# broadinstitute/Tangram

Measured on NVIDIA B200. Metric: map_cells_to_space iterations/sec, higher is better.
Workload: dtype bf16 operands / f32 accumulate+state

## Files before the change

tangram_b200/csrc/gemm_tc.cuh:

```cuda
#pragma once
#include <cuda.h>
#include <cstdio>
#include "common.cuh"
#include "gemm_simt.cuh"

namespace tgb {

constexpr int TC_BM = 128;
constexpr int TC_BK = 64;
constexpr int TC_UMMA_K = 16;
constexpr int TC_THREADS = 192;
constexpr int TC_RDOT_BN = 256;

__device__ __forceinline__ uint32_t smem_u32(const void* p) { return (uint32_t)__cvta_generic_to_shared(p); }

__device__ __forceinline__ void mbar_init(uint64_t* bar, uint32_t count) {
  asm volatile("mbarrier.init.shared::cta.b64 [%0], %1;" ::"r"(smem_u32(bar)), "r"(count));
}
__device__ __forceinline__ void mbar_expect_tx(uint64_t* bar, uint32_t bytes) {
  asm volatile("mbarrier.arrive.expect_tx.shared::cta.b64 _, [%0], %1;" ::"r"(smem_u32(bar)), "r"(bytes) : "memory");
}
__device__ __forceinline__ void mbar_wait(uint64_t* bar, uint32_t parity) {
  asm volatile(
      "{\n\t.reg .pred p;\n\t"
// ... 339 lines not shown
    }
  } else if (warp == 1) {
    if (lane == 0) {
      uint32_t kbg = 0;
      int it = 0;
      for (int w = blockIdx.x; w < total; w += gridDim.x, ++it) {
        const int z = w / (tiles_n * tiles_m);
        const int k_begin = k_off + z * k_per_split;
        const int k_end = min(k_total, k_begin + k_per_split);
        const int num_kb = (k_end - k_begin + TC_BK - 1) / TC_BK;
        const int b = it & 1;
        mbar_wait(&tempty_bar[b], (((uint32_t)it >> 1) & 1) ^ 1);
        tc_fence_after();
        const uint32_t d_tmem = tmem_base + (uint32_t)(b * BN);
        const int total_kb = num_kb * n_pairs;
        for (int kb = 0; kb < total_kb; ++kb, ++kbg) {
          const int s = kbg % STAGES;
          const uint32_t ph = (kbg / STAGES) & 1;
          mbar_wait(&full_bar[s], ph);
          tc_fence_after();
          const uint32_t sa = smem_u32(smem + s * kStageBytes);
          const uint32_t sb = sa + TileA::kBytes;
#pragma unroll
          for (int k = 0; k < TC_BK / TC_UMMA_K; ++k)
            umma_bf16(d_tmem, TileA::desc(sa, k), TileB::desc(sb, k), kIdesc, (kb > 0 || k > 0) ? 1u : 0u);
          umma_commit(&empty_bar[s]);
        }
        umma_commit(&tfull_bar[b]);
      }
    }
  } else {
    const int q = warp & 3;
    const int ew = warp - 2;
    int it = 0;
    for (int w = blockIdx.x; w < total; w += gridDim.x, ++it) {
      TileCoord t;
      t.split = w / (tiles_n * tiles_m);
      int tm_i;
      tile_mn(w - t.split * tiles_n * tiles_m, tiles_m, tiles_n, group_m, tm_i, t.tile_n);
      t.tiles_n = tiles_n;
      t.n0 = t.tile_n * BN;
      t.m0 = (tm_off + tm_i) * TC_BM;
      const int b = it & 1;
#ifndef TGB_SKIP_EPI
      epi.template prologue<BN, EPI_WARPS>(t, q, ew, lane);
#endif
      mbar_wait(&tfull_bar[b], ((uint32_t)it >> 1) & 1);
      tc_fence_after();
#ifndef TGB_SKIP_EPI
      epi.template run<BN, EPI_WARPS>(tmem_base + (uint32_t)(b * BN), q, ew, lane, t);
#endif
      tc_fence_before();
      __syncwarp();
      if (lane == 0) mbar_arrive(&tempty_bar[b]);
    }
    epi.finish(ew, lane, 0);
  }
  tc_fence_before();
  __syncthreads();
  if (warp == 1) tmem_dealloc(tmem_base, kTmemCols);
}

__device__ __forceinline__ uint32_t cluster_ctarank() {
  uint32_t r;
  asm volatile("mov.u32 %0, %%cluster_ctarank;" : "=r"(r));
  return r;
}
__device__ __forceinline__ void cluster_sync_all() {
  asm volatile("barrier.cluster.arrive.release.aligned;\n\tbarrier.cluster.wait.acquire.aligned;" ::: "memory");
}
__device__ __forceinline__ uint32_t mapa_shared(uint32_t addr, uint32_t rank) {
  uint32_t r;
  asm volatile("mapa.shared::cluster.u32 %0, %1, %2;" : "=r"(r) : "r"(addr), "r"(rank));
  return r;
}
__device__ __forceinline__ void mbar_arrive_remote(uint32_t cluster_addr) {
  asm volatile("mbarrier.arrive.release.cluster.shared::cluster.b64 _, [%0];" ::"r"(cluster_addr) : "memory");
}
__device__ __forceinline__ void tma_load_2d_pair(const CUtensorMap* map, uint32_t leader_bar, uint32_t dst, int c0, int c1, uint64_t policy) {
  asm volatile(
      "cp.async.bulk.tensor.2d.cta_group::2.shared::cluster.global.mbarrier::complete_tx::bytes.L2::cache_hint [%0], [%1, {%3, %4}], [%2], %5;"
      ::"r"(dst), "l"(map), "r"(leader_bar), "r"(c0), "r"(c1), "l"(policy) : "memory");
}
__device__ __forceinline__ void umma_bf16_pair(uint32_t d_tmem, uint64_t a_desc, uint64_t b_desc, uint32_t idesc, uint32_t accumulate) {
  asm volatile(
      "{\n\t.reg .pred p;\n\t"
      "setp.ne.b32 p, %4, 0;\n\t"
      "tcgen05.mma.cta_group::2.kind::f16 [%0], %1, %2, %3, p;\n\t}"
      ::"r"(d_tmem), "l"(a_desc), "l"(b_desc), "r"(idesc), "r"(accumulate) : "memory");
}
__device__ __forceinline__ void umma_commit_pair(uint64_t* bar) {
  asm volatile("tcgen05.commit.cta_group::2.mbarrier::arrive::one.shared::cluster.multicast::cluster.b64 [%0], %1;"
               ::"r"(smem_u32(bar)), "h"((uint16_t)3) : "memory");
}
__device__ __forceinline__ void tmem_alloc_pair(uint32_t* dst_smem, uint32_t ncols) {
  asm volatile("tcgen05.alloc.cta_group::2.sync.aligned.shared::cta.b32 [%0], %1;" ::"r"(smem_u32(dst_smem)), "r"(ncols) : "memory");
  asm volatile("tcgen05.relinquish_alloc_permit.cta_group::2.sync.aligned;" ::: "memory");
}
__device__ __forceinline__ void tmem_dealloc_pair(uint32_t taddr, uint32_t ncols) {
  asm volatile("tcgen05.dealloc.cta_group::2.sync.aligned.b32 %0, %1;" ::"r"(taddr), "r"(ncols) : "memory");
}

template <int BN, int STAGES, int EPI_WARPS, class Epi>
__global__ void __launch_bounds__(64 + 32 * EPI_WARPS, 1)
k_gemm_tc_pair(const __grid_constant__ TcMaps maps_a, const __grid_constant__ TcMaps maps_b, int n_pairs, int k_total, int tiles_m, int tiles_n, int group_m,
               uint64_t policy_a, uint64_t policy_b, int tm_off, const Epi epi) {
  using TileA = OperandTile<true, TC_BM>;
  using TileB = OperandTile<true, BN / 2>;
  constexpr int kStageBytes = TileA::kBytes + TileB::kBytes;
  constexpr uint32_t kTmemCols = 2 * BN;
  static_assert(kTmemCols == 256 || kTmemCols == 512, "TMEM allocation must be a power of two <= 512");
  constexpr uint32_t kIdesc = make_idesc(2 * TC_BM, BN, false, false);

  extern __shared__ uint8_t smem_raw[];
  uint8_t* smem = reinterpret_cast<uint8_t*>(((uintptr_t)smem_raw + 1023) & ~(uintptr_t)1023);
  __shared__ __align__(8) uint64_t full_bar[STAGES];
  __shared__ __align__(8) uint64_t empty_bar[STAGES];
  __shared__ __align__(8) uint64_t tfull_bar[2];
  __shared__ __align__(8) uint64_t tempty_bar[2];
  __shared__ uint32_t tmem_base_smem;

  const int warp = threadIdx.x >> 5, lane = threadIdx.x & 31;
  const uint32_t rank = cluster_ctarank();
  const int cid = blockIdx.x >> 1, ncl = gridDim.x >> 1;
  const int total = tiles_m * tiles_n;
  const int num_kb = (k_total + TC_BK - 1) / TC_BK;

  if (warp == 0 && lane == 0) {
    tma_prefetch_desc(&maps_a.m[0]);
    tma_prefetch_desc(&maps_b.m[0]);
#pragma unroll
    for (int s = 0; s < STAGES; ++s) { mbar_init(&full_bar[s], 1); mbar_init(&empty_bar[s], 1); }
#pragma unroll
    for (int b = 0; b < 2; ++b) { mbar_init(&tfull_bar[b], 1); mbar_init(&tempty_bar[b], 2 * EPI_WARPS); }
    fence_barrier_init();
  }
  if (warp == 1) tmem_alloc_pair(&tmem_base_smem, kTmemCols);
  tc_fence_before();
  cluster_sync_all();
  tc_fence_after();
  const uint32_t tmem_base = tmem_base_smem;

  if (warp == 0) {
#ifdef TGB_SKIP_MAINLOOP
    if (false) {
#else
    if (lane == 0) {
#endif
      uint32_t kbg = 0;
      for (int w = cid; w < total; w += ncl) {
        int tm_i, tn_i;
        tile_mn(w, tiles_m, tiles_n, group_m, tm_i, tn_i);
        const int n0 = tn_i * BN + (int)rank * (BN / 2);
        const int m0 = (tm_off + tm_i) * (2 * TC_BM) + (int)rank * TC_BM;
        for (int pr = 6 - n_pairs; pr < 6; ++pr) {
          const CUtensorMap* ma = &maps_a.m[kPairA[pr]];
          const CUtensorMap* mb = &maps_b.m[kPairB[pr]];
          for (int kb = 0; kb < num_kb; ++kb, ++kbg) {
            const int s = kbg % STAGES;
            const uint32_t ph = (kbg / STAGES) & 1;
            mbar_wait(&empty_bar[s], ph ^ 1);
            const uint32_t sa = smem_u32(smem + s * kStageBytes);
            const uint32_t sb = sa + TileA::kBytes;
            if (rank == 0) mbar_expect_tx(&full_bar[s], 2 * kStageBytes);
            const uint32_t lbar = mapa_shared(smem_u32(&full_bar[s]), 0);
            tma_load_2d_pair(ma, lbar, sa, kb * TC_BK, m0, policy_a);
            tma_load_2d_pair(mb, lbar, sb, kb * TC_BK, n0, policy_b);
          }
        }
      }
    }
  } else if (warp == 1) {
    if (lane == 0 && rank == 0) {
      uint32_t kbg = 0;
      int it = 0;
      for (int w = cid; w < total; w += ncl, ++it) {
        const int b = it & 1;
        mbar_wait(&tempty_bar[b], (((uint32_t)it >> 1) & 1) ^ 1);
        tc_fence_after();
        const uint32_t d_tmem = tmem_base + (uint32_t)(b * BN);
#ifdef TGB_SKIP_MAINLOOP
        const int total_kb = 0;
#else
        const int total_kb = num_kb * n_pairs;
#endif
        for (int kb = 0; kb < total_kb; ++kb, ++kbg) {
          const int s = kbg % STAGES;
          const uint32_t ph = (kbg / STAGES) & 1;
          mbar_wait(&full_bar[s], ph);
          tc_fence_after();
          const uint32_t sa = smem_u32(smem + s * kStageBytes);
          const uint32_t sb = sa + TileA::kBytes;
#pragma unroll
          for (int k = 0; k < TC_BK / TC_UMMA_K; ++k)
            umma_bf16_pair(d_tmem, TileA::desc(sa, k), TileB::desc(sb, k), kIdesc, (kb > 0 || k > 0) ? 1u : 0u);
          umma_commit_pair(&empty_bar[s]);
        }
        umma_commit_pair(&tfull_bar[b]);
      }
    }
  } else {
    const int q = warp & 3;
    const int ew = warp - 2;
    const uint32_t tempty_remote = mapa_shared(smem_u32(&tempty_bar[0]), 0);
    int it = 0;
    for (int w = cid; w < total; w += ncl, ++it) {
      TileCoord t;
      int tm_i;
      tile_mn(w, tiles_m, tiles_n, group_m, tm_i, t.tile_n);
      t.tiles_n = tiles_n;
      t.n0 = t.tile_n * BN;
      t.m0 = (tm_off + tm_i) * (2 * TC_BM) + (int)rank * TC_BM;
      t.split = 0;
      const int b = it & 1;
#ifndef TGB_SKIP_EPI
      epi.template prologue<BN, EPI_WARPS>(t, q, ew, lane);
#endif
      mbar_wait(&tfull_bar[b], ((uint32_t)it >> 1) & 1);
      tc_fence_after();
#ifndef TGB_SKIP_EPI
      epi.template run<BN, EPI_WARPS>(tmem_base + (uint32_t)(b * BN), q, ew, lane, t);
#endif
      tc_fence_before();
      __syncwarp();
      if (lane == 0) mbar_arrive_remote(tempty_remote + (uint32_t)b * 8u);
    }
    epi.finish(ew, lane, 0);
  }
  tc_fence_before();
  cluster_sync_all();
  if (warp == 1) tmem_dealloc_pair(tmem_base, kTmemCols);
}

typedef CUresult (*PFN_encodeTiled)(CUtensorMap*, CUtensorMapDataType, cuuint32_t, void*, const cuuint64_t*,
                                    const cuuint64_t*, const cuuint32_t*, const cuuint32_t*, CUtensorMapInterleave,
                                    CUtensorMapSwizzle, CUtensorMapL2promotion, CUtensorMapFloatOOBfill);

struct TcContext {
  PFN_encodeTiled encode = nullptr;
  int num_sms = 148;
  int pair_clusters = -1;
  int dp_clusters = -1;
  const void* smem_fn[16] = {};
  int smem_bytes[16] = {};
};

static inline int tc_init(TcContext& tc, char* err, size_t n) {
  void* fn = nullptr;
  cudaDriverEntryPointQueryResult qres;
  cudaError_t e = cudaGetDriverEntryPoint("cuTensorMapEncodeTiled", &fn, cudaEnableDefault, &qres);
  if (e != cudaSuccess || fn == nullptr || qres != cudaDriverEntryPointSuccess) {
    snprintf(err, n, "cuTensorMapEncodeTiled not available from the driver (%s)", cudaGetErrorString(e));
    return -2;
  }
  tc.encode = (PFN_encodeTiled)fn;
  int dev = 0;
  cudaGetDevice(&dev);
  cudaDeviceGetAttribute(&tc.num_sms, cudaDevAttrMultiProcessorCount, dev);
  return 0;
}

static inline int tc_make_map(TcContext& tc, CUtensorMap* map, const void* base, uint64_t cols, uint64_t rows,
                              uint64_t ld, uint32_t box_inner, uint32_t box_outer, char* err, size_t n) {
  cuuint64_t dims[2] = {cols, rows};
  cuuint64_t strides[1] = {ld * 2};
  cuuint32_t box[2] = {box_inner, box_outer};
  cuuint32_t estr[2] = {1, 1};
  CUresult r = tc.encode(map, CU_TENSOR_MAP_DATA_TYPE_BFLOAT16, 2, const_cast<void*>(base), dims, strides, box, estr,
                         CU_TENSOR_MAP_INTERLEAVE_NONE, CU_TENSOR_MAP_SWIZZLE_128B, CU_TENSOR_MAP_L2_PROMOTION_L2_256B,
                         CU_TENSOR_MAP_FLOAT_OOB_FILL_NONE);
  if (r != CUDA_SUCCESS) {
    snprintf(err, n, "cuTensorMapEncodeTiled failed (%d) cols=%llu rows=%llu ld=%llu box=%ux%u", (int)r,
             (unsigned long long)cols, (unsigned long long)rows, (unsigned long long)ld, box_inner, box_outer);
    return -2;
  }
  return 0;
}

template <class Kern>
static inline int tc_set_smem(TcContext& tc, Kern kern, int bytes, char* err, size_t n) {
  const void* key = reinterpret_cast<const void*>(kern);
  int slot = -1;
  for (int i = 0; i < 16; ++i) {
    if (tc.smem_fn[i] == key) { if (tc.smem_bytes[i] == bytes) return 0; slot = i; break; }
    if (tc.smem_fn[i] == nullptr && slot < 0) slot = i;
  }
  cudaError_t e = cudaFuncSetAttribute(kern, cudaFuncAttributeMaxDynamicSharedMemorySize, bytes);
  if (e != cudaSuccess) { snprintf(err, n, "cudaFuncSetAttribute(smem=%d): %s", bytes, cudaGetErrorString(e)); return -2; }
  if (slot >= 0) { tc.smem_fn[slot] = key; tc.smem_bytes[slot] = bytes; }
  return 0;
}
static inline int tc_check_launch(const char* name, char* err, size_t n) {
  cudaError_t e = cudaGetLastError();
  if (e != cudaSuccess) { snprintf(err, n, "launch %s: %s", name, cudaGetErrorString(e)); return -2; }
  return 0;
}

constexpr int TC_FWD_BN = 256, TC_FWD_STAGES = 4;
#ifndef TGB_BWD_BN
#define TGB_BWD_BN 256
#endif
constexpr int TC_BWD_BN = TGB_BWD_BN;
#ifndef TGB_BWD_PAIR
#define TGB_BWD_PAIR 1
#endif
constexpr int TC_PAIR_MIN_ROWS = 2048;
#ifndef TGB_DP_STAGES
#define TGB_DP_STAGES 6
#endif
#ifndef TGB_DP_EPI_WARPS
#define TGB_DP_EPI_WARPS 4
#endif
constexpr int TC_DP_STAGES = TGB_DP_STAGES, TC_DP_SINGLE_STAGES = 4, TC_DP_EPI_WARPS = TGB_DP_EPI_WARPS;
static inline int tc_dp_row_parts(int V) { return (int)ceil_div(V, TC_BWD_BN) * (TC_DP_EPI_WARPS / 4); }
static inline int tc_splits(long long tiles, long long k_total, int min_k) {
  long long s = (2 * 148 + tiles - 1) / tiles;
  const long long max_s = (k_total + min_k - 1) / min_k;
  if (s > max_s) s = max_s;
  if (s < 1) s = 1;
  const long long kps = ((k_total + s - 1) / s + TC_BK - 1) / TC_BK * TC_BK;
  return (int)((k_total + kps - 1) / kps);
}
static inline int tc_splits_for_chain(long long k_total, int max_chain) {
  long long s = (k_total + max_chain - 1) / max_chain;
  if (s < 1) s = 1;
  const long long kps = ((k_total + s - 1) / s + TC_BK - 1) / TC_BK * TC_BK;
  return (int)((k_total + kps - 1) / kps);
}
static inline int tc_forward_splits(int N, int V, int Ke) {
  return tc_splits((long long)ceil_div(V, TC_BM) * ceil_div(Ke, TC_FWD_BN), N, 512);
}
static inline int tc_kps(int k_total, int splits) {
  return (int)(round_up(ceil_div(k_total, splits), TC_BK));
}
static inline unsigned tc_grid(const TcContext& tc, long long total) {
  return (unsigned)(total < tc.num_sms ? total : tc.num_sms);
}

static inline int tc_make_maps(TcContext& tc, TcMaps* maps, const __nv_bfloat16* base, size_t plane_elems, int n_planes,
                               uint64_t cols, uint64_t rows, uint64_t ld, uint32_t bi, uint32_t bo, char* err, size_t n) {
  for (int p = 0; p < 3; ++p) {
    const __nv_bfloat16* ptr = base + (size_t)(p < n_planes ? p : 0) * plane_elems;
    if (tc_make_map(tc, &maps->m[p], ptr, cols, rows, ld, bi, bo, err, n)) return -2;
  }
  return 0;
}

struct TcPlan {
  TcMaps a, b;
  bool pair = false;
  bool ready = false;
};

static inline int tc_forward_plan(TcContext& tc, TcPlan& pl, const __nv_bfloat16* P, size_t p_plane, const __nv_bfloat16* Sx,
                                  size_t s_plane, int planes, int N, int V, int Ke, int ld, char* err, size_t n) {
  if (tc_make_maps(tc, &pl.a, P, p_plane, planes, V, N, ld, 64, 64, err, n)) return -2;
  if (tc_make_maps(tc, &pl.b, Sx, s_plane, planes, Ke, N, Ke, 64, 64, err, n)) return -2;
  pl.ready = true;
  return 0;
}
static inline int tc_forward_launch(TcContext& tc, const TcPlan& pl, int n_pairs, float* out, int N, int V, int Ke, int splits,
                                    cudaStream_t s, char* err, size_t n) {
  auto kern = k_gemm_tc<false, false, TC_FWD_BN, TC_FWD_STAGES, 4, TcEpiStore>;
  const int smem = TC_FWD_STAGES * (TC_BM + TC_FWD_BN) * TC_BK * 2 + 1024;
  if (tc_set_smem(tc, kern, smem, err, n)) return -2;
  TcEpiStore epi{out, Ke, (size_t)V * Ke, V, 0};
  const int tm = (int)ceil_div(V, TC_BM), tn = (int)ceil_div(Ke, TC_FWD_BN);
  kern<<<tc_grid(tc, (long long)tm * tn * splits), 64 + 32 * 4, smem, s>>>(pl.a, pl.b, n_pairs, N, tc_kps(N, splits), tm, tn,
                                                                         splits, 1, kPolicyEvictNormal, kPolicyEvictNormal, 0, 0, epi);
  return tc_check_launch("tc_gemm_fwd", err, n);
}
static inline int tc_forward_launch_rows(TcContext& tc, const TcPlan& pl, float* out, int accumulate, int row0, int row1, int V, int Ke,
                                         cudaStream_t s, char* err, size_t n) {
  auto kern = k_gemm_tc<false, false, TC_FWD_BN, TC_FWD_STAGES, 4, TcEpiStore>;
  const int smem = TC_FWD_STAGES * (TC_BM + TC_FWD_BN) * TC_BK * 2 + 1024;
  if (tc_set_smem(tc, kern, smem, err, n)) return -2;
  TcEpiStore epi{out, Ke, (size_t)V * Ke, V, accumulate};
  const int tm = (int)ceil_div(V, TC_BM), tn = (int)ceil_div(Ke, TC_FWD_BN);
  kern<<<tc_grid(tc, (long long)tm * tn), 64 + 32 * 4, smem, s>>>(pl.a, pl.b, 1, row1, (int)round_up(row1 - row0, TC_BK), tm, tn,
                                                                1, 1, kPolicyEvictNormal, kPolicyEvictNormal, 0, row0, epi);
  return tc_check_launch("tc_gemm_fwd", err, n);
}
static inline int tc_forward(TcContext& tc, const __nv_bfloat16* P, size_t p_plane, const __nv_bfloat16* Sx, size_t s_plane,
                             int n_pairs, float* out, int N, int V, int Ke, int ld, int splits, cudaStream_t s, char* err,
                             size_t n) {
  TcPlan pl;
  if (tc_forward_plan(tc, pl, P, p_plane, Sx, s_plane, n_pairs > 1 ? 3 : 1, N, V, Ke, ld, err, n)) return -2;
  return tc_forward_launch(tc, pl, n_pairs, out, N, V, Ke, splits, s, err, n);
}

template <class Kern>
static inline int tc_pair_clusters(TcContext& tc, Kern pk, int threads, int smem, cudaStream_t s) {
  cudaLaunchConfig_t cfg = {};
  cfg.blockDim = dim3(threads); cfg.dynamicSmemBytes = smem; cfg.stream = s;
  cudaLaunchAttribute at[1];
  at[0].id = cudaLaunchAttributeClusterDimension;
  at[0].val.clusterDim.x = 2; at[0].val.clusterDim.y = 1; at[0].val.clusterDim.z = 1;
  cfg.attrs = at; cfg.numAttrs = 1;
  cfg.gridDim = dim3(tc.num_sms & ~1);
  int mc = 0;
  const int r = cudaOccupancyMaxActiveClusters(&mc, pk, &cfg) == cudaSuccess ? mc : 0;
  (void)cudaGetLastError();
  return r;
}
template <class Kern, class... Args>
static inline cudaError_t tc_launch_pair(Kern pk, unsigned clusters, int threads, int smem, cudaStream_t s, Args... args) {
  cudaLaunchConfig_t cfg = {};
  cfg.blockDim = dim3(threads); cfg.dynamicSmemBytes = smem; cfg.stream = s;
  cudaLaunchAttribute at[1];
  at[0].id = cudaLaunchAttributeClusterDimension;
  at[0].val.clusterDim.x = 2; at[0].val.clusterDim.y = 1; at[0].val.clusterDim.z = 1;
  cfg.attrs = at; cfg.numAttrs = 1;
  cfg.gridDim = dim3(2 * clusters);
  return cudaLaunchKernelEx(&cfg, pk, args...);
}

template <class Epi>
static inline int tc_dpstore_plan(TcContext& tc, TcPlan& pl, const __nv_bfloat16* Sxb, size_t s_plane, const __nv_bfloat16* dYb,
                                  size_t dy_plane, int planes, int N, int V, int Ke, cudaStream_t s, char* err, size_t n) {
  if (tc_make_maps(tc, &pl.a, Sxb, s_plane, planes, Ke, N, Ke, 64, TC_BM, err, n)) return -2;
  pl.pair = false;
#if TGB_BWD_PAIR
  if (N >= TC_PAIR_MIN_ROWS) {
    auto pk = k_gemm_tc_pair<TC_BWD_BN, TC_DP_STAGES, TC_DP_EPI_WARPS, Epi>;
    const int psmem = TC_DP_STAGES * (TC_BM + TC_BWD_BN / 2) * TC_BK * 2 + 1024;
    if (tc_set_smem(tc, pk, psmem, err, n)) return -2;
    if (tc.dp_clusters < 0) tc.dp_clusters = tc_pair_clusters(tc, pk, 64 + 32 * TC_DP_EPI_WARPS, psmem, s);
    pl.pair = tc.dp_clusters > 0;
  }
#endif
  if (tc_make_maps(tc, &pl.b, dYb, dy_plane, planes, Ke, V, Ke, 64, pl.pair ? TC_BWD_BN / 2 : TC_BWD_BN, err, n)) return -2;
  pl.ready = true;
  return 0;
}
template <class Epi>
static inline int tc_dpstore_launch(TcContext& tc, const TcPlan& pl, int n_pairs, const Epi& epi, int row0, int row1, int V, int Ke,
                                    cudaStream_t s, char* err, size_t n) {
  const int tn = (int)ceil_div(V, TC_BWD_BN);
  if (pl.pair) {
    auto pk = k_gemm_tc_pair<TC_BWD_BN, TC_DP_STAGES, TC_DP_EPI_WARPS, Epi>;
    const int psmem = TC_DP_STAGES * (TC_BM + TC_BWD_BN / 2) * TC_BK * 2 + 1024;
    const int tm0 = row0 / (2 * TC_BM), tmp = (int)ceil_div(row1, 2 * TC_BM) - tm0;
    const long long pair_tiles = (long long)tmp * tn;
    const unsigned clusters = (unsigned)(pair_tiles < tc.dp_clusters ? pair_tiles : tc.dp_clusters);
    cudaError_t e = tc_launch_pair(pk, clusters, 64 + 32 * TC_DP_EPI_WARPS, psmem, s, pl.a, pl.b, n_pairs, Ke, tmp, tn, 1,
                                   (uint64_t)kPolicyEvictNormal, (uint64_t)kPolicyEvictLast, tm0, epi);
    if (e != cudaSuccess) { snprintf(err, n, "launch tc_gemm_bwd_dp (pair): %s", cudaGetErrorString(e)); return -2; }
    return tc_check_launch("tc_gemm_bwd_dp", err, n);
  }
  auto kern = k_gemm_tc<true, true, TC_BWD_BN, TC_DP_SINGLE_STAGES, TC_DP_EPI_WARPS, Epi>;
  const int smem = TC_DP_SINGLE_STAGES * (TC_BM + TC_BWD_BN) * TC_BK * 2 + 1024;
  if (tc_set_smem(tc, kern, smem, err, n)) return -2;
  const int tm0 = row0 / TC_BM, tm = (int)ceil_div(row1, TC_BM) - tm0;
  kern<<<tc_grid(tc, (long long)tm * tn), 64 + 32 * TC_DP_EPI_WARPS, smem, s>>>(pl.a, pl.b, n_pairs, Ke, Ke, tm, tn, 1, 1,
                                                                                kPolicyEvictNormal, kPolicyEvictLast, tm0, 0, epi);
  return tc_check_launch("tc_gemm_bwd_dp", err, n);
}

}
```

tangram_b200/csrc/tangram_b200.cu:

```cuda
#include "../../include/tangram_b200.h"

#include <cmath>
#include <cstdarg>
#include <cstdio>
#include <cstdlib>
#include <cstring>
#include <string>
#include <thread>
#include <vector>

#include "common.cuh"
#include "kernels_elem.cuh"
#include "gemm_simt.cuh"
#include "gemm_tc.cuh"
#include "adam_rows.cuh"
#include "nccl_dl.h"

using namespace tgb;

static thread_local char g_err[1024] = "";
static int fail(int code, const char* fmt, ...) {
  va_list ap;
  va_start(ap, fmt);
  vsnprintf(g_err, sizeof(g_err), fmt, ap);
// ... 273 lines not shown
    if (nc < 1) nc = 1;
    if (nc > 8) nc = 8;
    if (h->constrained) nc = 1;
    while (nc > 1 && h->N / nc < 1024) --nc;
    h->nchunks = nc;
    for (int c = 0; c <= nc; ++c) h->chunk_row[c] = c == nc ? h->N : (int)round_up((int64_t)c * h->N / nc, 256);
  }
  if (h->staged && h->nchunks > 1) {
    int lo_p = 0, hi_p = 0;
    cudaDeviceGetStreamPriorityRange(&lo_p, &hi_p);
    const int mid_p = hi_p < lo_p ? hi_p + 1 : lo_p;
    bool ok = cudaStreamCreateWithPriority(&h->hi, cudaStreamNonBlocking, hi_p) == cudaSuccess &&
              cudaStreamCreateWithPriority(&h->sf, cudaStreamNonBlocking, mid_p) == cudaSuccess &&
              cudaStreamCreateWithPriority(&h->lo, cudaStreamNonBlocking, lo_p) == cudaSuccess;
    cudaEvent_t* evs[5] = {&h->ev_fork, &h->ev_join_hi, &h->ev_join_lo, &h->ev_join_sf, &h->ev_loss};
    for (auto e : evs) ok = ok && cudaEventCreateWithFlags(e, cudaEventDisableTiming) == cudaSuccess;
    for (int c = 0; c < 8; ++c)
      ok = ok && cudaEventCreateWithFlags(&h->ev_g[c], cudaEventDisableTiming) == cudaSuccess &&
           cudaEventCreateWithFlags(&h->ev_a[c], cudaEventDisableTiming) == cudaSuccess &&
           cudaEventCreateWithFlags(&h->ev_f[c], cudaEventDisableTiming) == cudaSuccess;
    if (!ok) A(fail(TGB200_ERR_CUDA, "stream / event creation failed: %s", cudaGetErrorString(cudaGetLastError())));
    h->pipelined = ok;
    h->l2_persist = getenv("TGB200_L2_PERSIST") && atoi(getenv("TGB200_L2_PERSIST")) != 0;
  }
  {
    const int tiles = (int)(ceil_div(h->V, 128) * ceil_div(h->Ke, 128));
    int s = (int)ceil_div(2 * 148, tiles);
    const int max_s = (int)ceil_div(h->N, 512);
    if (s > max_s) s = max_s;
    if (s < 1) s = 1;
    if (h->tcm) s = tc_forward_splits(h->N, h->V, h->Ke);
    if (h->x3) { const int c = tc_splits_for_chain(h->N, 2048); if (c > s) s = c; }
    if (h->nchunks > 1) s = 1;
    h->fwd_splits = s;
    if (s > 1) A(h->Ypart.alloc((size_t)s * vk));
  }
  A(h->Y.alloc(vk + kTail)); A(h->dY.alloc(vk));
  if (h->constrained) {
    A(h->Fl.alloc(h->N)); A(h->mF.alloc(h->N)); A(h->vF.alloc(h->N)); A(h->fsig.alloc(h->N));
    A(h->Sf.alloc((size_t)h->N * h->Ke)); A(h->fscal.alloc(4));
  }
  h->r_parts = h->tcm ? tc_dp_row_parts(h->V) : (int)ceil_div(h->Ke, SG_BN);
  A(h->rpart.alloc((size_t)h->r_parts * h->N));
  A(h->ngc.alloc(h->Ke)); A(h->ngr.alloc(h->V));
  h->loss_rows = 16;
  while (ceil_div(h->V, h->loss_rows) > 512 && h->loss_rows < kLossRowsMax) h->loss_rows += 16;
  h->nchunk = (int)ceil_div(h->V, h->loss_rows);
  A(h->colfin.alloc((size_t)7 * h->Ke));
  h->ncolchunk = (int)ceil_div(h->Ke, kLossCols);
  h->nredchunk = (int)ceil_div(h->Ke, kLossColsBlk);
  A(h->colpart.alloc((size_t)h->nchunk * 3 * h->Ke));
  A(h->coefA.alloc(h->Ke)); A(h->coefB.alloc(h->Ke));
  A(h->densg.alloc(h->V));
  if (cfg->lambda_g2 != 0.f) { A(h->rowpart.alloc((size_t)h->ncolchunk * h->V * 2)); A(h->coefAr.alloc(h->V)); A(h->coefBr.alloc(h->V)); }
  if (cfg->lambda_neighborhood_g1 > 0.f) {
    A(h->WG.alloc(vk)); A(h->nwg.alloc(h->Ke)); A(h->Z.alloc(vk)); A(h->colpart_nb.alloc((size_t)h->nchunk * 2 * h->Ke));
    A(h->coefAn.alloc(h->Ke)); A(h->coefBn.alloc(h->Ke));
  }
  if (cfg->lambda_getis_ord > 0.f) {
    A(h->AG.alloc(vk)); A(h->nag.alloc(h->Ke)); A(h->sgnG.alloc(h->Ke)); A(h->Zg.alloc(vk));
    A(h->colpart_go.alloc((size_t)h->nchunk * 2 * h->Ke)); A(h->coefAg.alloc(h->Ke)); A(h->coefBg.alloc(h->Ke));
  }
  if (cfg->lambda_ct_islands > 0.f) {
    h->n_ct_blocks = (int)ceil_div((int64_t)h->V * h->T, 256);
    A(h->H.alloc((size_t)h->V * h->T)); A(h->ctpart.alloc(h->n_ct_blocks));
  }
  if (st == TGB200_OK && h->l2_persist && h->pipelined) {
    const size_t bytes = (size_t)h->V * h->Ke * sizeof(__nv_bfloat16);
    int max_persist = 0, max_window = 0;
    cudaDeviceGetAttribute(&max_persist, cudaDevAttrMaxPersistingL2CacheSize, cfg->device);
    cudaDeviceGetAttribute(&max_window, cudaDevAttrMaxAccessPolicyWindowSize, cfg->device);
    const size_t want = bytes < (size_t)max_persist ? bytes : (size_t)max_persist;
    cudaDeviceSetLimit(cudaLimitPersistingL2CacheSize, want);
    cudaStreamAttrValue attr = {};
    attr.accessPolicyWindow.base_ptr = h->dYb.p;
    attr.accessPolicyWindow.num_bytes = bytes < (size_t)max_window ? bytes : (size_t)max_window;
    attr.accessPolicyWindow.hitRatio = want >= bytes ? 1.0f : (float)want / (float)bytes;
    attr.accessPolicyWindow.hitProp = cudaAccessPropertyPersisting;
    attr.accessPolicyWindow.missProp = cudaAccessPropertyStreaming;
    if (cudaStreamSetAttribute(h->hi, cudaStreamAttributeAccessPolicyWindow, &attr) != cudaSuccess) { (void)cudaGetLastError(); h->l2_persist = false; }
  }
  if (st == TGB200_OK && h->tcm) st = tc_init(h->tc, g_err, sizeof(g_err));
  if (st != TGB200_OK) { delete h; return st; }
  CK(cudaDeviceSynchronize());
  *out = h;
  return TGB200_OK;
}

extern "C" int tgb200_destroy(tgb200_mapper* h) {
  if (!h) return TGB200_OK;
  cudaSetDevice(h->cfg.device);
  cudaDeviceSynchronize();
  delete h;
  return TGB200_OK;
}

static int upload_padded(tgb200_mapper* h, const float* src, int rows, int cols, float* dst, int ld, int col_off,
                         cudaStream_t s) {
  DevBuf<float> tmp;
  CKS(tmp.alloc((size_t)rows * cols, false));
  CK(cudaMemcpyAsync(tmp.p, src, (size_t)rows * cols * sizeof(float), cudaMemcpyDefault, s));
  const long long n = (long long)rows * cols;
  k_pack_rows<<<(unsigned)ceil_div(n, 256), 256, 0, s>>>(tmp.p, rows, cols, dst, ld, col_off);
  LAUNCH_CHECK("pack_rows");
  CK(cudaStreamSynchronize(s));
  return TGB200_OK;
}

static int refresh_bf16_operands(tgb200_mapper* h, cudaStream_t s) {
  if (!h->tcm) return TGB200_OK;
  const long long n = (long long)h->N * h->Ke;
  if (h->x3) {
    k_split3<<<(unsigned)ceil_div(n / 4, 256), 256, 0, s>>>(s_act(h), Split3{h->Sxb.p, (size_t)n}, n / 4);
    LAUNCH_CHECK("split3");
    return TGB200_OK;
  }
  k_f32_to_bf16<<<(unsigned)ceil_div(n, 256), 256, 0, s>>>(s_act(h), h->Sxb.p, n);
  LAUNCH_CHECK("f32_to_bf16");
  return TGB200_OK;
}

static int fill_density_cols(tgb200_mapper* h, cudaStream_t s) {
  const float* w = (h->cfg.density_mode == TGB200_DENSITY_SOURCE) ? h->dsrc.p : nullptr;
  k_fill_density_cols<<<(unsigned)ceil_div(h->N, 256), 256, 0, s>>>(h->Sx.p, h->N, h->Ke, h->K, w, h->bf16 ? 1 : 0);
  LAUNCH_CHECK("fill_density_cols");
  return refresh_bf16_operands(h, s);
}

static int precompute_graph_constants(tgb200_mapper* h, cudaStream_t s) {
  if (!h->have_expr) return TGB200_OK;
  dim3 grid(h->V, (unsigned)ceil_div(h->Ke, 128));
  if (h->cfg.lambda_neighborhood_g1 > 0.f && h->W.set) {
    k_spmm<<<grid, 128, 0, s>>>(h->V, h->K, h->Ke, h->W.view(), h->G.p, h->WG.p);
    LAUNCH_CHECK("spmm");
    k_col_norms<<<(unsigned)ceil_div(h->K, 128), 128, 0, s>>>(h->V, h->K, h->Ke, h->WG.p, h->nwg.p, nullptr);
    LAUNCH_CHECK("col_norms");
  }
  if (h->cfg.lambda_getis_ord > 0.f && h->A.set) {
    k_spmm<<<grid, 128, 0, s>>>(h->V, h->K, h->Ke, h->A.view(), h->G.p, h->AG.p);
    LAUNCH_CHECK("spmm");
    k_col_norms<<<(unsigned)ceil_div(h->K, 128), 128, 0, s>>>(h->V, h->K, h->Ke, h->AG.p, h->nag.p, nullptr);
    LAUNCH_CHECK("col_norms");
    k_col_norms<<<(unsigned)ceil_div(h->K, 128), 128, 0, s>>>(h->V, h->K, h->Ke, h->G.p, h->ngc.p, h->sgnG.p);
    LAUNCH_CHECK("col_norms");
  }
  return TGB200_OK;
}

extern "C" int tgb200_set_expression(tgb200_mapper* h, const float* S, const float* G, void* stream) {
  if (!h || !S || !G) return fail(TGB200_ERR_INVALID, "null argument");
  cudaStream_t s = (cudaStream_t)stream;
  CK(cudaSetDevice(h->cfg.device));
  CK(cudaMemsetAsync(h->Sx.p, 0, h->Sx.n * sizeof(float), s));
  CK(cudaMemsetAsync(h->G.p, 0, h->G.n * sizeof(float), s));
  CKS(upload_padded(h, S, h->N, h->K, h->Sx.p, h->Ke, 0, s));
  CKS(upload_padded(h, G, h->V, h->K, h->G.p, h->Ke, 0, s));
  k_col_norms<<<(unsigned)ceil_div(h->K, 128), 128, 0, s>>>(h->V, h->K, h->Ke, h->G.p, h->ngc.p, nullptr);
  LAUNCH_CHECK("col_norms");
  k_row_norms<<<(unsigned)ceil_div(h->V, 8), 256, 0, s>>>(h->V, h->K, h->Ke, h->G.p, h->ngr.p);
  LAUNCH_CHECK("row_norms");
  h->have_expr = true;
  h->have_ct = false;
  CKS(fill_density_cols(h, s));
  CKS(precompute_graph_constants(h, s));
  CK(cudaStreamSynchronize(s));
  return TGB200_OK;
// ... 961 lines not shown
```

Before: 102.6.

## Use 2-CTA pair kernel for forward GEMM and add 4-CTA TMA multicast

Generalizes the cta_group::2 tensor-core kernel to support MN-major operands, a K offset, and 4-CTA clusters in which two CTA pairs share one operand through TMA multicast. The forward GEMM now uses the pair kernel with optional multicast of A across adjacent N tiles, and the backward dP GEMM can multicast B across adjacent M tiles. The aim is fewer global/L2 operand loads and larger effective tiles. In exchange it adds cluster-wide empty-barrier arrivals, idle half-tiles when the tile count is odd, and possibly lower occupancy with 4-CTA clusters.

Measured after the change: 104.1 (median of 6 runs). Within noise of the previous version (+1.5%).

```diff
diff --git a/tangram_b200/csrc/gemm_tc.cuh b/tangram_b200/csrc/gemm_tc.cuh
--- a/tangram_b200/csrc/gemm_tc.cuh
+++ b/tangram_b200/csrc/gemm_tc.cuh
@@ -445,6 +445,13 @@
       "cp.async.bulk.tensor.2d.cta_group::2.shared::cluster.global.mbarrier::complete_tx::bytes.L2::cache_hint [%0], [%1, {%3, %4}], [%2], %5;"
       ::"r"(dst), "l"(map), "r"(leader_bar), "r"(c0), "r"(c1), "l"(policy) : "memory");
 }
+__device__ __forceinline__ void tma_load_2d_pair_mc(const CUtensorMap* map, uint32_t leader_bar, uint32_t dst, int c0, int c1, uint64_t policy,
+                                                    uint16_t mask) {
+  asm volatile(
+      "cp.async.bulk.tensor.2d.cta_group::2.shared::cluster.global.mbarrier::complete_tx::bytes.multicast::cluster.L2::cache_hint"
+      " [%0], [%1, {%3, %4}], [%2], %5, %6;"
+      ::"r"(dst), "l"(map), "r"(leader_bar), "r"(c0), "r"(c1), "h"(mask), "l"(policy) : "memory");
+}
 __device__ __forceinline__ void umma_bf16_pair(uint32_t d_tmem, uint64_t a_desc, uint64_t b_desc, uint32_t idesc, uint32_t accumulate) {
   asm volatile(
       "{\n\t.reg .pred p;\n\t"
@@ -452,9 +459,9 @@
       "tcgen05.mma.cta_group::2.kind::f16 [%0], %1, %2, %3, p;\n\t}"
       ::"r"(d_tmem), "l"(a_desc), "l"(b_desc), "r"(idesc), "r"(accumulate) : "memory");
 }
-__device__ __forceinline__ void umma_commit_pair(uint64_t* bar) {
+__device__ __forceinline__ void umma_commit_pair(uint64_t* bar, uint16_t mask) {
   asm volatile("tcgen05.commit.cta_group::2.mbarrier::arrive::one.shared::cluster.multicast::cluster.b64 [%0], %1;"
-               ::"r"(smem_u32(bar)), "h"((uint16_t)3) : "memory");
+               ::"r"(smem_u32(bar)), "h"(mask) : "memory");
 }
 __device__ __forceinline__ void tmem_alloc_pair(uint32_t* dst_smem, uint32_t ncols) {
   asm volatile("tcgen05.alloc.cta_group::2.sync.aligned.shared::cta.b32 [%0], %1;" ::"r"(smem_u32(dst_smem)), "r"(ncols) : "memory");
@@ -464,16 +471,34 @@
   asm volatile("tcgen05.dealloc.cta_group::2.sync.aligned.b32 %0, %1;" ::"r"(taddr), "r"(ncols) : "memory");
 }
 
-template <int BN, int STAGES, int EPI_WARPS, class Epi>
+template <bool KMAJOR, int ROWS>
+__device__ __forceinline__ void pair_load(const CUtensorMap* map, uint32_t lbar, uint32_t dst, int mn0, int k0, uint64_t policy) {
+  if (KMAJOR) {
+    tma_load_2d_pair(map, lbar, dst, k0, mn0, policy);
+  } else {
+#pragma unroll
+    for (int b = 0; b < ROWS / 64; ++b) tma_load_2d_pair(map, lbar, dst + b * 8192, mn0 + b * 64, k0, policy);
+  }
+}
+template <bool KMAJOR>
+__device__ __forceinline__ void pair_load_mc(const CUtensorMap* map, uint32_t lbar, uint32_t dst, int mn0, int k0, uint64_t policy,
+                                             uint16_t mask) {
+  if (KMAJOR) tma_load_2d_pair_mc(map, lbar, dst, k0, mn0, policy, mask);
+  else tma_load_2d_pair_mc(map, lbar, dst, mn0, k0, policy, mask);
+}
+
+template <bool A_KMAJOR, bool B_KMAJOR, int BN, int STAGES, int EPI_WARPS, int MC, class Epi>
 __global__ void __launch_bounds__(64 + 32 * EPI_WARPS, 1)
-k_gemm_tc_pair(const __grid_constant__ TcMaps maps_a, const __grid_constant__ TcMaps maps_b, int n_pairs, int k_total, int tiles_m, int tiles_n, int group_m,
-               uint64_t policy_a, uint64_t policy_b, int tm_off, const Epi epi) {
-  using TileA = OperandTile<true, TC_BM>;
-  using TileB = OperandTile<true, BN / 2>;
-  constexpr int kStageBytes = TileA::kBytes + TileB::kBytes;
+k_gemm_tc_pair(const __grid_constant__ TcMaps maps_a, const __grid_constant__ TcMaps maps_b, int n_pairs, int k_off, int k_total,
+               int tiles_m, int tiles_n, int group_m, uint64_t policy_a, uint64_t policy_b, int tm_off, const Epi epi) {
+  constexpr int CL = MC ? 4 : 2;
+  constexpr int kBytesA = TC_BM * TC_BK * 2;
+  constexpr int kBytesB = BN / 2 * TC_BK * 2;
+  constexpr int kStageBytes = kBytesA + kBytesB;
   constexpr uint32_t kTmemCols = 2 * BN;
   static_assert(kTmemCols == 256 || kTmemCols == 512, "TMEM allocation must be a power of two <= 512");
-  constexpr uint32_t kIdesc = make_idesc(2 * TC_BM, BN, false, false);
+  static_assert(BN / 2 == TC_BM || MC != 2, "multicast of B splits a 128-row half tile");
+  constexpr uint32_t kIdesc = make_idesc(2 * TC_BM, BN, !A_KMAJOR, !B_KMAJOR);
 
   extern __shared__ uint8_t smem_raw[];
   uint8_t* smem = reinterpret_cast<uint8_t*>(((uintptr_t)smem_raw + 1023) & ~(uintptr_t)1023);
@@ -485,15 +510,23 @@
 
   const int warp = threadIdx.x >> 5, lane = threadIdx.x & 31;
   const uint32_t rank = cluster_ctarank();
-  const int cid = blockIdx.x >> 1, ncl = gridDim.x >> 1;
-  const int total = tiles_m * tiles_n;
-  const int num_kb = (k_total + TC_BK - 1) / TC_BK;
+  const uint32_t pr = rank & 1, pp = rank >> 1;
+  const uint32_t leader = rank & ~1u;
+  const int cid = blockIdx.x / CL, ncl = gridDim.x / CL;
+  const int items_m = MC == 2 ? (tiles_m + 1) / 2 : tiles_m, items_n = MC == 1 ? (tiles_n + 1) / 2 : tiles_n;
+  const int total = items_m * items_n;
+  const int num_kb = (k_total - k_off + TC_BK - 1) / TC_BK;
+  auto my_tile = [&](int w, int& tm_i, int& tn_i) {
+    tile_mn(w, items_m, items_n, group_m, tm_i, tn_i);
+    if (MC == 1) tn_i = 2 * tn_i + (int)pp;
+    if (MC == 2) tm_i = 2 * tm_i + (int)pp;
+  };
 
   if (warp == 0 && lane == 0) {
     tma_prefetch_desc(&maps_a.m[0]);
     tma_prefetch_desc(&maps_b.m[0]);
 #pragma unroll
-    for (int s = 0; s < STAGES; ++s) { mbar_init(&full_bar[s], 1); mbar_init(&empty_bar[s], 1); }
+    for (int s = 0; s < STAGES; ++s) { mbar_init(&full_bar[s], 1); mbar_init(&empty_bar[s], MC ? 2 : 1); }
 #pragma unroll
     for (int b = 0; b < 2; ++b) { mbar_init(&tfull_bar[b], 1); mbar_init(&tempty_bar[b], 2 * EPI_WARPS); }
     fence_barrier_init();
@@ -510,31 +543,37 @@
 #else
     if (lane == 0) {
 #endif
+      const uint16_t mc_mask = (uint16_t)((1u << pr) | (1u << (2 + pr)));
       uint32_t kbg = 0;
       for (int w = cid; w < total; w += ncl) {
         int tm_i, tn_i;
-        tile_mn(w, tiles_m, tiles_n, group_m, tm_i, tn_i);
-        const int n0 = tn_i * BN + (int)rank * (BN / 2);
-        const int m0 = (tm_off + tm_i) * (2 * TC_BM) + (int)rank * TC_BM;
-        for (int pr = 6 - n_pairs; pr < 6; ++pr) {
-          const CUtensorMap* ma = &maps_a.m[kPairA[pr]];
-          const CUtensorMap* mb = &maps_b.m[kPairB[pr]];
+        my_tile(w, tm_i, tn_i);
+        const int n0 = tn_i * BN + (int)pr * (BN / 2);
+        const int m0 = (tm_off + tm_i) * (2 * TC_BM) + (int)pr * TC_BM;
+        for (int prr = 6 - n_pairs; prr < 6; ++prr) {
+          const CUtensorMap* ma = &maps_a.m[kPairA[prr]];
+          const CUtensorMap* mb = &maps_b.m[kPairB[prr]];
           for (int kb = 0; kb < num_kb; ++kb, ++kbg) {
             const int s = kbg % STAGES;
             const uint32_t ph = (kbg / STAGES) & 1;
             mbar_wait(&empty_bar[s], ph ^ 1);
             const uint32_t sa = smem_u32(smem + s * kStageBytes);
-            const uint32_t sb = sa + TileA::kBytes;
-            if (rank == 0) mbar_expect_tx(&full_bar[s], 2 * kStageBytes);
-            const uint32_t lbar = mapa_shared(smem_u32(&full_bar[s]), 0);
-            tma_load_2d_pair(ma, lbar, sa, kb * TC_BK, m0, policy_a);
-            tma_load_2d_pair(mb, lbar, sb, kb * TC_BK, n0, policy_b);
+            const uint32_t sb = sa + kBytesA;
+            if (pr == 0) mbar_expect_tx(&full_bar[s], 2 * kStageBytes);
+            const uint32_t lbar = mapa_shared(smem_u32(&full_bar[s]), leader);
+            const int k0 = k_off + kb * TC_BK;
+            if (MC == 1) pair_load_mc<A_KMAJOR>(ma, lbar, sa + pp * 8192, m0 + (int)pp * 64, k0, policy_a, mc_mask);
+            else pair_load<A_KMAJOR, TC_BM>(ma, lbar, sa, m0, k0, policy_a);
+            if (MC == 2) pair_load_mc<B_KMAJOR>(mb, lbar, sb + pp * 8192, n0 + (int)pp * 64, k0, policy_b, mc_mask);
+            else pair_load<B_KMAJOR, BN / 2>(mb, lbar, sb, n0, k0, policy_b);
           }
         }
       }
     }
   } else if (warp == 1) {
-    if (lane == 0 && rank == 0) {
+    if (lane == 0 && pr == 0) {
+      const uint16_t pair_mask = (uint16_t)(3u << (2 * pp));
+      const uint16_t empty_mask = MC ? (uint16_t)0xF : (uint16_t)3;
       uint32_t kbg = 0;
       int it = 0;
       for (int w = cid; w < total; w += ncl, ++it) {
@@ -553,36 +592,38 @@
           mbar_wait(&full_bar[s], ph);
           tc_fence_after();
           const uint32_t sa = smem_u32(smem + s * kStageBytes);
-          const uint32_t sb = sa + TileA::kBytes;
+          const uint32_t sb = sa + kBytesA;
 #pragma unroll
           for (int k = 0; k < TC_BK / TC_UMMA_K; ++k)
-            umma_bf16_pair(d_tmem, TileA::desc(sa, k), TileB::desc(sb, k), kIdesc, (kb > 0 || k > 0) ? 1u : 0u);
-          umma_commit_pair(&empty_bar[s]);
+            umma_bf16_pair(d_tmem, OperandTile<A_KMAJOR, TC_BM>::desc(sa, k), OperandTile<B_KMAJOR, BN / 2>::desc(sb, k), kIdesc,
+                           (kb > 0 || k > 0) ? 1u : 0u);
+          umma_commit_pair(&empty_bar[s], empty_mask);
         }
-        umma_commit_pair(&tfull_bar[b]);
+        umma_commit_pair(&tfull_bar[b], pair_mask);
       }
     }
   } else {
     const int q = warp & 3;
     const int ew = warp - 2;
-    const uint32_t tempty_remote = mapa_shared(smem_u32(&tempty_bar[0]), 0);
+    const uint32_t tempty_remote = mapa_shared(smem_u32(&tempty_bar[0]), leader);
     int it = 0;
     for (int w = cid; w < total; w += ncl, ++it) {
       TileCoord t;
       int tm_i;
-      tile_mn(w, tiles_m, tiles_n, group_m, tm_i, t.tile_n);
+      my_tile(w, tm_i, t.tile_n);
+      const bool live = tm_i < tiles_m && t.tile_n < tiles_n;
       t.tiles_n = tiles_n;
       t.n0 = t.tile_n * BN;
-      t.m0 = (tm_off + tm_i) * (2 * TC_BM) + (int)rank * TC_BM;
+      t.m0 = (tm_off + tm_i) * (2 * TC_BM) + (int)pr * TC_BM;
       t.split = 0;
       const int b = it & 1;
 #ifndef TGB_SKIP_EPI
-      epi.template prologue<BN, EPI_WARPS>(t, q, ew, lane);
+      if (live) epi.template prologue<BN, EPI_WARPS>(t, q, ew, lane);
 #endif
       mbar_wait(&tfull_bar[b], ((uint32_t)it >> 1) & 1);
       tc_fence_after();
 #ifndef TGB_SKIP_EPI
-      epi.template run<BN, EPI_WARPS>(tmem_base + (uint32_t)(b * BN), q, ew, lane, t);
+      if (live) epi.template run<BN, EPI_WARPS>(tmem_base + (uint32_t)(b * BN), q, ew, lane, t);
 #endif
       tc_fence_before();
       __syncwarp();
@@ -602,8 +643,12 @@
 struct TcContext {
   PFN_encodeTiled encode = nullptr;
   int num_sms = 148;
-  int pair_clusters = -1;
   int dp_clusters = -1;
+  int dp_mc_clusters = -1;
+  int fwd_clusters = -1;
+  int fwd_mc_clusters = -1;
+  bool fwd_pair = true;
+  int multicast = 3;
   const void* smem_fn[16] = {};
   int smem_bytes[16] = {};
 };
@@ -712,6 +757,7 @@
 struct TcPlan {
   TcMaps a, b;
   bool pair = false;
+  bool mc = false;
   bool ready = false;
 };
 
@@ -733,17 +779,6 @@
                                                                          splits, 1, kPolicyEvictNormal, kPolicyEvictNormal, 0, 0, epi);
   return tc_check_launch("tc_gemm_fwd", err, n);
 }
-static inline int tc_forward_launch_rows(TcContext& tc, const TcPlan& pl, float* out, int accumulate, int row0, int row1, int V, int Ke,
-                                         cudaStream_t s, char* err, size_t n) {
-  auto kern = k_gemm_tc<false, false, TC_FWD_BN, TC_FWD_STAGES, 4, TcEpiStore>;
-  const int smem = TC_FWD_STAGES * (TC_BM + TC_FWD_BN) * TC_BK * 2 + 1024;
-  if (tc_set_smem(tc, kern, smem, err, n)) return -2;
-  TcEpiStore epi{out, Ke, (size_t)V * Ke, V, accumulate};
-  const int tm = (int)ceil_div(V, TC_BM), tn = (int)ceil_div(Ke, TC_FWD_BN);
-  kern<<<tc_grid(tc, (long long)tm * tn), 64 + 32 * 4, smem, s>>>(pl.a, pl.b, 1, row1, (int)round_up(row1 - row0, TC_BK), tm, tn,
-                                                                1, 1, kPolicyEvictNormal, kPolicyEvictNormal, 0, row0, epi);
-  return tc_check_launch("tc_gemm_fwd", err, n);
-}
 static inline int tc_forward(TcContext& tc, const __nv_bfloat16* P, size_t p_plane, const __nv_bfloat16* Sx, size_t s_plane,
                              int n_pairs, float* out, int N, int V, int Ke, int ld, int splits, cudaStream_t s, char* err,
                              size_t n) {
@@ -753,29 +788,73 @@
 }
 
 template <class Kern>
-static inline int tc_pair_clusters(TcContext& tc, Kern pk, int threads, int smem, cudaStream_t s) {
+static inline int tc_pair_clusters(TcContext& tc, Kern pk, int csize, int threads, int smem, cudaStream_t s) {
   cudaLaunchConfig_t cfg = {};
   cfg.blockDim = dim3(threads); cfg.dynamicSmemBytes = smem; cfg.stream = s;
   cudaLaunchAttribute at[1];
   at[0].id = cudaLaunchAttributeClusterDimension;
-  at[0].val.clusterDim.x = 2; at[0].val.clusterDim.y = 1; at[0].val.clusterDim.z = 1;
+  at[0].val.clusterDim.x = csize; at[0].val.clusterDim.y = 1; at[0].val.clusterDim.z = 1;
   cfg.attrs = at; cfg.numAttrs = 1;
-  cfg.gridDim = dim3(tc.num_sms & ~1);
+  cfg.gridDim = dim3(tc.num_sms / csize * csize);
   int mc = 0;
   const int r = cudaOccupancyMaxActiveClusters(&mc, pk, &cfg) == cudaSuccess ? mc : 0;
   (void)cudaGetLastError();
   return r;
 }
 template <class Kern, class... Args>
-static inline cudaError_t tc_launch_pair(Kern pk, unsigned clusters, int threads, int smem, cudaStream_t s, Args... args) {
+static inline cudaError_t tc_launch_pair(Kern pk, int csize, unsigned clusters, int threads, int smem, cudaStream_t s, Args... args) {
   cudaLaunchConfig_t cfg = {};
   cfg.blockDim = dim3(threads); cfg.dynamicSmemBytes = smem; cfg.stream = s;
   cudaLaunchAttribute at[1];
   at[0].id = cudaLaunchAttributeClusterDimension;
-  at[0].val.clusterDim.x = 2; at[0].val.clusterDim.y = 1; at[0].val.clusterDim.z = 1;
+  at[0].val.clusterDim.x = csize; at[0].val.clusterDim.y = 1; at[0].val.clusterDim.z = 1;
   cfg.attrs = at; cfg.numAttrs = 1;
-  cfg.gridDim = dim3(2 * clusters);
+  cfg.gridDim = dim3(csize * clusters);
   return cudaLaunchKernelEx(&cfg, pk, args...);
+}
+
+static inline int tc_forward_launch_rows(TcContext& tc, const TcPlan& pl, float* out, int accumulate, int row0, int row1, int V, int Ke,
+                                         cudaStream_t s, char* err, size_t n) {
+  TcEpiStore epi{out, Ke, (size_t)V * Ke, V, accumulate};
+  const int kb_len = (int)round_up(row1 - row0, TC_BK);
+  if (tc.fwd_pair) {
+    constexpr int kStages = TC_DP_STAGES;
+    const int psmem = kStages * (TC_BM + TC_FWD_BN / 2) * TC_BK * 2 + 1024;
+    const int tm = (int)ceil_div(V, 2 * TC_BM), tn = (int)ceil_div(Ke, TC_FWD_BN);
+    auto pk = k_gemm_tc_pair<false, false, TC_FWD_BN, kStages, 4, 0, TcEpiStore>;
+    auto mk = k_gemm_tc_pair<false, false, TC_FWD_BN, kStages, 4, 1, TcEpiStore>;
+    if (tc.fwd_clusters < 0) {
+      if (tc_set_smem(tc, pk, psmem, err, n)) return -2;
+      tc.fwd_clusters = tc_pair_clusters(tc, pk, 2, 64 + 32 * 4, psmem, s);
+      tc.fwd_mc_clusters = 0;
+      if (tc.multicast & 1) {
+        if (tc_set_smem(tc, mk, psmem, err, n)) return -2;
+        tc.fwd_mc_clusters = tc_pair_clusters(tc, mk, 4, 64 + 32 * 4, psmem, s);
+      }
+    }
+    const long long pair_tiles = (long long)tm * tn;
+    if (tc.fwd_clusters > 0 && pair_tiles >= tc.fwd_clusters) {
+      cudaError_t e;
+      if (tc.fwd_mc_clusters > 0) {
+        const long long items = (long long)tm * ((tn + 1) / 2);
+        const unsigned clusters = (unsigned)(items < tc.fwd_mc_clusters ? items : tc.fwd_mc_clusters);
+        e = tc_launch_pair(mk, 4, clusters, 64 + 32 * 4, psmem, s, pl.a, pl.b, 1, row0, row0 + kb_len, tm, tn, 1,
+                           (uint64_t)kPolicyEvictNormal, (uint64_t)kPolicyEvictNormal, 0, epi);
+      } else {
+        e = tc_launch_pair(pk, 2, (unsigned)tc.fwd_clusters, 64 + 32 * 4, psmem, s, pl.a, pl.b, 1, row0, row0 + kb_len, tm, tn, 1,
+                           (uint64_t)kPolicyEvictNormal, (uint64_t)kPolicyEvictNormal, 0, epi);
+      }
+      if (e != cudaSuccess) { snprintf(err, n, "launch tc_gemm_fwd (pair): %s", cudaGetErrorString(e)); return -2; }
+      return tc_check_launch("tc_gemm_fwd", err, n);
+    }
+  }
+  auto kern = k_gemm_tc<false, false, TC_FWD_BN, TC_FWD_STAGES, 4, TcEpiStore>;
+  const int smem = TC_FWD_STAGES * (TC_BM + TC_FWD_BN) * TC_BK * 2 + 1024;
+  if (tc_set_smem(tc, kern, smem, err, n)) return -2;
+  const int tm = (int)ceil_div(V, TC_BM), tn = (int)ceil_div(Ke, TC_FWD_BN);
+  kern<<<tc_grid(tc, (long long)tm * tn), 64 + 32 * 4, smem, s>>>(pl.a, pl.b, 1, row1, kb_len, tm, tn,
+                                                                1, 1, kPolicyEvictNormal, kPolicyEvictNormal, 0, row0, epi);
+  return tc_check_launch("tc_gemm_fwd", err, n);
 }
 
 template <class Epi>
@@ -783,16 +862,24 @@
                                   size_t dy_plane, int planes, int N, int V, int Ke, cudaStream_t s, char* err, size_t n) {
   if (tc_make_maps(tc, &pl.a, Sxb, s_plane, planes, Ke, N, Ke, 64, TC_BM, err, n)) return -2;
   pl.pair = false;
+  pl.mc = false;
 #if TGB_BWD_PAIR
   if (N >= TC_PAIR_MIN_ROWS) {
-    auto pk = k_gemm_tc_pair<TC_BWD_BN, TC_DP_STAGES, TC_DP_EPI_WARPS, Epi>;
     const int psmem = TC_DP_STAGES * (TC_BM + TC_BWD_BN / 2) * TC_BK * 2 + 1024;
+    auto pk = k_gemm_tc_pair<true, true, TC_BWD_BN, TC_DP_STAGES, TC_DP_EPI_WARPS, 0, Epi>;
     if (tc_set_smem(tc, pk, psmem, err, n)) return -2;
-    if (tc.dp_clusters < 0) tc.dp_clusters = tc_pair_clusters(tc, pk, 64 + 32 * TC_DP_EPI_WARPS, psmem, s);
+    if (tc.dp_clusters < 0) tc.dp_clusters = tc_pair_clusters(tc, pk, 2, 64 + 32 * TC_DP_EPI_WARPS, psmem, s);
     pl.pair = tc.dp_clusters > 0;
-  }
-#endif
-  if (tc_make_maps(tc, &pl.b, dYb, dy_plane, planes, Ke, V, Ke, 64, pl.pair ? TC_BWD_BN / 2 : TC_BWD_BN, err, n)) return -2;
+    if (pl.pair && (tc.multicast & 2) && planes == 1) {
+      auto mk = k_gemm_tc_pair<true, true, TC_BWD_BN, TC_DP_STAGES, TC_DP_EPI_WARPS, 2, Epi>;
+      if (tc_set_smem(tc, mk, psmem, err, n)) return -2;
+      if (tc.dp_mc_clusters < 0) tc.dp_mc_clusters = tc_pair_clusters(tc, mk, 4, 64 + 32 * TC_DP_EPI_WARPS, psmem, s);
+      pl.mc = tc.dp_mc_clusters > 0;
+    }
+  }
+#endif
+  const uint32_t b_rows = pl.mc ? TC_BWD_BN / 4 : (pl.pair ? TC_BWD_BN / 2 : TC_BWD_BN);
+  if (tc_make_maps(tc, &pl.b, dYb, dy_plane, planes, Ke, V, Ke, 64, b_rows, err, n)) return -2;
   pl.ready = true;
   return 0;
 }
@@ -801,13 +888,22 @@
                                     cudaStream_t s, char* err, size_t n) {
   const int tn = (int)ceil_div(V, TC_BWD_BN);
   if (pl.pair) {
-    auto pk = k_gemm_tc_pair<TC_BWD_BN, TC_DP_STAGES, TC_DP_EPI_WARPS, Epi>;
     const int psmem = TC_DP_STAGES * (TC_BM + TC_BWD_BN / 2) * TC_BK * 2 + 1024;
     const int tm0 = row0 / (2 * TC_BM), tmp = (int)ceil_div(row1, 2 * TC_BM) - tm0;
-    const long long pair_tiles = (long long)tmp * tn;
-    const unsigned clusters = (unsigned)(pair_tiles < tc.dp_clusters ? pair_tiles : tc.dp_clusters);
-    cudaError_t e = tc_launch_pair(pk, clusters, 64 + 32 * TC_DP_EPI_WARPS, psmem, s, pl.a, pl.b, n_pairs, Ke, tmp, tn, 1,
-                                   (uint64_t)kPolicyEvictNormal, (uint64_t)kPolicyEvictLast, tm0, epi);
+    cudaError_t e;
+    if (pl.mc) {
+      auto mk = k_gemm_tc_pair<true, true, TC_BWD_BN, TC_DP_STAGES, TC_DP_EPI_WARPS, 2, Epi>;
+      const long long items = (long long)((tmp + 1) / 2) * tn;
+      const unsigned clusters = (unsigned)(items < tc.dp_mc_clusters ? items : tc.dp_mc_clusters);
+      e = tc_launch_pair(mk, 4, clusters, 64 + 32 * TC_DP_EPI_WARPS, psmem, s, pl.a, pl.b, n_pairs, 0, Ke, tmp, tn, 1,
+                         (uint64_t)kPolicyEvictNormal, (uint64_t)kPolicyEvictLast, tm0, epi);
+    } else {
+      auto pk = k_gemm_tc_pair<true, true, TC_BWD_BN, TC_DP_STAGES, TC_DP_EPI_WARPS, 0, Epi>;
+      const long long pair_tiles = (long long)tmp * tn;
+      const unsigned clusters = (unsigned)(pair_tiles < tc.dp_clusters ? pair_tiles : tc.dp_clusters);
+      e = tc_launch_pair(pk, 2, clusters, 64 + 32 * TC_DP_EPI_WARPS, psmem, s, pl.a, pl.b, n_pairs, 0, Ke, tmp, tn, 1,
+                         (uint64_t)kPolicyEvictNormal, (uint64_t)kPolicyEvictLast, tm0, epi);
+    }
     if (e != cudaSuccess) { snprintf(err, n, "launch tc_gemm_bwd_dp (pair): %s", cudaGetErrorString(e)); return -2; }
     return tc_check_launch("tc_gemm_bwd_dp", err, n);
   }
diff --git a/tangram_b200/csrc/tangram_b200.cu b/tangram_b200/csrc/tangram_b200.cu
--- a/tangram_b200/csrc/tangram_b200.cu
+++ b/tangram_b200/csrc/tangram_b200.cu
@@ -379,6 +379,8 @@
   }
   if (st == TGB200_OK && h->tcm) st = tc_init(h->tc, g_err, sizeof(g_err));
   if (st != TGB200_OK) { delete h; return st; }
+  h->tc.fwd_pair = !(getenv("TGB200_FWD_PAIR") && atoi(getenv("TGB200_FWD_PAIR")) == 0);
+  if (const char* e = getenv("TGB200_TC_MULTICAST")) h->tc.multicast = atoi(e) & 3;
   CK(cudaDeviceSynchronize());
   *out = h;
   return TGB200_OK;
```
